# natir/yacrd

Hardware: AMD Instinct MI355X
Metric: reads_per_sec_classified (higher is better)
Workload: dtype u32

## Files before the change

include/yacrd_engine_debug.h:

```cpp
#ifndef YACRD_ENGINE_DEBUG_H
#define YACRD_ENGINE_DEBUG_H

#include "yacrd_engine.h"

#define YACRD_F_FORCE_GENERAL 1u
#define YACRD_F_FORCE_LDS_SORT 2u
#define YACRD_F_WAVE_ONLY 8u
#define YACRD_F_NO_HALVES 16u
#define YACRD_F_NO_PREDICTION 64u
#define YACRD_F_NO_PREFILTER 256u
#define YACRD_F_COUNT_PREFILTERED 512u
#define YACRD_F_NO_DEFER 4096u
#define YACRD_F_ALWAYS_DEFER 8192u
#define YACRD_F_SCREEN_ITEMS_1 262144u
#define YACRD_F_SCREEN_ITEMS_2 524288u
#define YACRD_F_NO_FUSED_SCREEN 1048576u
#define YACRD_F_STREAM_SCREEN 65536u
#define YACRD_F_SCREEN_WIDE 2097152u
#define YACRD_F_SCREEN_DIRECT 8388608u
#define YACRD_F_NO_SCREEN_DIRECT 16777216u

#ifdef __cplusplus
extern "C" {
#endif
int yacrd_debug_sort_pairs(yacrd_engine *e, uint64_t *keys, uint32_t *vals, uint64_t n, uint64_t key_bound);
uint64_t yacrd_debug_last_counters(const yacrd_engine *e, void *dst, uint64_t bytes);
int yacrd_debug_last_input_csr(yacrd_engine *e, uint64_t *n_reads, uint64_t *n_intervals, uint64_t *offsets, uint32_t *intervals,
                               uint32_t *lengths);
void yacrd_debug_peer_copy_counts(uint64_t out[3]);
void yacrd_debug_live_bytes(uint64_t out[2]);
uint64_t yacrd_debug_direct_runs(const yacrd_engine *e);
void yacrd_debug_big_routes(const yacrd_engine *e, uint64_t out[4]);
#ifdef __cplusplus
}
#endif

#endif
```

yacrd_amd/__init__.py:

```python
from .engine import (
    Engine, EngineError, NeedsHostParser, Result, lib_path, load_library, build, partition_reads, run_partitioned, ingest_overlaps,
    NOT_BAD, CHIMERIC, NOT_COVERED, TYPE_NAMES, F_FORCE_GENERAL, F_FORCE_LDS_SORT, F_WAVE_ONLY, F_NO_HALVES, F_TIMING_FULL, F_NO_PREDICTION, F_NO_PREFILTER, F_COUNT_PREFILTERED, F_NO_TIMING, F_BLOCKING_WAIT, F_NO_DEFER, F_ALWAYS_DEFER, F_TIMING_SAMPLED, F_STREAM_SCREEN, F_SCREEN_ITEMS_1, F_SCREEN_ITEMS_2, F_NO_FUSED_SCREEN, F_SCREEN_WIDE, F_ONE_LAUNCH, F_SCREEN_DIRECT, F_NO_SCREEN_DIRECT, DEBUG_SYMBOLS, run_device_batches, DeviceBatch,
    EXPORTED_SYMBOLS, CLASS_NAMES, CLASS_KERNELS, PinnedArray, Stream, StreamGroup, stream_device_of, HANDLE_ELSEWHERE, RecSink, OvlRec, OVL_REC_DTYPE, GzipWriter, ByteSink,
)
```

yacrd_amd/csrc/engine.hip:

```cpp
#include "engine_internal.h"

#include <time.h>

#include <algorithm>
#include <cstdio>
#include <cstdlib>
#include <cstring>
#include <string>
#include <thread>
#include <vector>

#include "device_common.h"
#include "plan_compact.h"
#include "sweep_big.h"
#include "sweep_wave.h"
#include "sweep_big_trim.h"
#include "sweep_general.h"
#include "sweep_lds.h"
#include "finish_compact.h"
#include "screen_wg.h"
#include "screen_stream.h"
#include "screen_big.h"
#include "one_batch.h"

using namespace yke;

static uint64_t env_u64(const char *name, uint64_t dflt)
{
    const char *v = std::getenv(name);
    return v ? std::strtoull(v, nullptr, 10) : dflt;
}

static uint64_t defer_min_intervals()
{
    static const uint64_t v = env_u64("YACRD_DEFER_MIN_IV", 4000000ull);
    return v;
}
static constexpr uint32_t kProbeEvery = 16;

static uint64_t split_min_reads()
{
    static const uint64_t v = env_u64("YACRD_SPLIT_MIN_READS", (uint64_t)yk::kPlanSmallReads);
    return v;
}

static uint64_t fused_share_override()
{
    static const uint64_t v = std::min<uint64_t>(env_u64("YACRD_FUSED_SHARE", 0), 4096);
    return v;
}
static uint64_t fused_grid_mult()
{
    static const uint64_t v = std::max<uint64_t>(1, env_u64("YACRD_TEST_FUSED_GRID_MULT", 1));
    return v;
}

namespace yke {
std::string &err_slot()
{
    thread_local std::string s;
    return s;
}
}

namespace {

yk::SweepArgs base_sweep_args(const yacrd_engine *e, const Run &R)
{
    yk::SweepArgs sa;
    sa.off = R.d_off, sa.iv = R.d_iv, sa.len = R.d_len, sa.cov = R.cov, sa.prefilter = R.prefilter;
    sa.list = nullptr, sa.list_n = nullptr, sa.rec = nullptr, sa.first = 0;
    sa.stage = e->stage.as<uint2>(), sa.counts = e->counts.as<u32>(), sa.closed = e->closed.as<uint2>(), sa.ctr = R.ctr;
    sa.rej_list = R.rej_small, sa.rej_count = &R.ctr->rej_small;
    sa.over_list = R.over_med, sa.over_count = &R.ctr->over_med;
    return sa;
}
yk::SweepArgs list_sweep_args(const Run &R, const u32 *list, const u32 *list_n)
{
    yk::SweepArgs sa = R.base;
    sa.list = list;
    sa.list_n = list_n;
    return sa;
}

yk::CompactArgs2 compact_args(const yacrd_engine *e, const Run &R)
{
    yk::CompactArgs2 ca;
    ca.sweep = R.base;
    ca.sweep.over_list = nullptr;
    ca.sweep.over_count = nullptr;
    ca.scan_state = reinterpret_cast<u64 *>(R.ctr + 1);
    ca.n_reads = R.n_reads;
    ca.not_cov = R.not_cov;
    ca.bad_offsets = e->bad_offsets.as<u64>();
    ca.bad_regions = e->bad_regions.as<uint2>();
    ca.region_cap = (u64)(e->bad_regions.cap / sizeof(uint2));
    ca.read_type = e->read_type.as<uint8_t>();
    ca.host_ctr = e->h_ctr();
    return ca;
}

int launch_compact(yacrd_engine *e, const Run &R)
{
    const u32 n_reads = R.n_reads;
    const yk::CompactArgs2 ca = compact_args(e, R);
    if (R.n_reads64 >= split_min_reads()) {
        if (R.screened) {
            const u32 slabs = (n_reads + yk::kMarkReads - 1) / yk::kMarkReads;
            yk::DeferList dl;
            dl.shard_cap = (slabs / yk::kDeferShards + 1u) * (u32)yk::kMarkReads;
            HIP_TRY(e->dlist.reserve((size_t)yk::kDeferShards * dl.shard_cap * sizeof(u32)));
            dl.list = e->dlist.as<u32>();
            dl.count = reinterpret_cast<u32 *>(ca.scan_state + R.nb);
            if (e->compact_calls++)
                HIP_TRY(hipMemsetAsync(dl.count, 0, (size_t)yk::kDeferShards * yk::kDeferShardStride * sizeof(u32), e->stream));
            hipLaunchKernelGGL(yk::mark_list_kernel, dim3(slabs), dim3(yk::kMarkThreads), 0, e->stream, ca.sweep.counts, n_reads, dl);
            hipLaunchKernelGGL(yk::deferred_list_kernel, dim3((u32)e->num_cu * (u32)(YK_LIST_OCC * 256 / yk::kListThreads)), dim3(yk::kListThreads), 0,
                               e->stream, ca.sweep, dl);
        }
        hipLaunchKernelGGL(yk::scan_compact_kernel<4>, dim3((n_reads + 4 * yk::kScanThreads - 1) / (4 * yk::kScanThreads)), dim3(yk::kScanThreads), 0, e->stream, ca);
        return YACRD_OK;
    }
    hipLaunchKernelGGL(yk::finish_compact_kernel, dim3((n_reads + yk::kScanBlock - 1) / yk::kScanBlock), dim3(yk::kScanBlock), 0, e->stream, ca);
    return YACRD_OK;
}

int gather_reads(yacrd_engine *e, const u64 *d_off, const u32 *d_len, const u32 *d_list, u32 count,
                 hipStream_t stream, std::vector<yk::GatherOut> &out)
{
    HIP_TRY(e->gen_sizes.reserve((size_t)count * sizeof(yk::GatherOut)));
    hipLaunchKernelGGL(yk::gather_general_sizes_kernel, dim3((count + 255) / 256), dim3(256), 0,
                       stream, d_off, d_len, d_list, count, e->gen_sizes.as<yk::GatherOut>());
    out.resize(count);
    HIP_TRY(hipMemcpyAsync(out.data(), e->gen_sizes.p, (size_t)count * sizeof(yk::GatherOut),
                           hipMemcpyDeviceToHost, stream));
    HIP_TRY(hipStreamSynchronize(stream));
    for (const auto &g : out)
        if (g.n >= 0x7FFFFFFFull) return fail(YACRD_EINVAL, "a read has >= 2^31 - 1 intervals");
    return YACRD_OK;
}

int run_general_global(yacrd_engine *e, const u64 *d_off, const uint2 *d_iv, const u32 *d_len,
                       const u32 *d_list, u32 count, u32 cov, hipStream_t stream)
{
    std::vector<yk::GatherOut> info;
    int rc = gather_reads(e, d_off, d_len, d_list, count, stream, info);
    if (rc) return rc;
    for (const auto &g : info)
        if (2 * g.n > (u64)yk::kMedium2Events) e->big_routes[3]++;
    HIP_TRY(e->gen_scratch_off.reserve((size_t)count * sizeof(u64)));
    std::vector<u64> offs(count);
    u64 tot = 0;
    for (u32 i = 0; i < count; i++) {
        offs[i] = tot;
        tot += 3 * info[i].n + 2;
    }
    HIP_TRY(e->gen_scratch.reserve((size_t)tot * sizeof(u64)));
    HIP_TRY(hipMemcpyAsync(e->gen_scratch_off.p, offs.data(), (size_t)count * sizeof(u64),
                           hipMemcpyHostToDevice, stream));
    HIP_TRY(hipStreamSynchronize(stream));
    yk::GeneralArgs ga;
    ga.off = d_off;
    ga.iv = d_iv;
    ga.len = d_len;
    ga.list = d_list;
    ga.scratch_off = e->gen_scratch_off.as<u64>();
    ga.scratch = e->gen_scratch.as<u64>();
    ga.cov = cov;
    ga.stage = e->stage.as<uint2>();
    ga.counts = e->counts.as<u32>();
    hipLaunchKernelGGL(yk::sweep_general_kernel, dim3(count), dim3(yk::kGenThreads), 0, stream, ga);
    return YACRD_OK;
}
// ... 129 lines not shown
        std::vector<yk::GatherOut> rest;
        for (u32 i = 0; i < count; i++) {
            if (bs[i].flags & yk::BT_TRIMMED) {
                e->big_routes[1]++;
                continue;
            }
            if (bs[i].flags & yk::BT_BAD) redo.push_back(info[i].read);
            else rest.push_back(info[i]);
        }
        info.swap(rest);
        count = (u32)info.size();
    }
    if (count) {
        rc = run_big_sort(e, d_iv, info, cov, stream, redo);
        if (rc) return rc;
    }
    if (!redo.empty()) {
        HIP_TRY(e->big_redo.reserve(redo.size() * sizeof(u32)));
        HIP_TRY(hipMemcpyAsync(e->big_redo.p, redo.data(), redo.size() * sizeof(u32),
                               hipMemcpyHostToDevice, stream));
        HIP_TRY(hipStreamSynchronize(stream));
        rc = run_general_global(e, d_off, d_iv, d_len, e->big_redo.as<u32>(), (u32)redo.size(), cov, stream);
        if (rc) return rc;
    }
    return YACRD_OK;
}

int wait_for_stream(yacrd_engine *e)
{
    if (e->flags & YACRD_F_BLOCKING_WAIT) {
        HIP_TRY(hipEventRecord(e->ev_sync[EVS_DONE], e->stream));
        for (;;) {
            const hipError_t q = hipEventQuery(e->ev_sync[EVS_DONE]);
            if (q == hipSuccess) break;
            if (q != hipErrorNotReady) HIP_TRY(q);
            struct timespec ts = {0, 20000};
            nanosleep(&ts, nullptr);
        }
    } else {
        HIP_TRY(hipStreamSynchronize(e->stream));
    }
    HIP_TRY(hipGetLastError());
    return YACRD_OK;
}

int conclude_run(yacrd_engine *e, const Run &R, float extra_ms);
int finish_pending(yacrd_engine *e);


int reserve_buffers(yacrd_engine *e, Run &R)
{
    const u32 n_reads = R.n_reads;
    const uint64_t n_reads64 = R.n_reads64;
    R.ob_slabs = (n_reads + yk::kObSlab - 1) / yk::kObSlab;
    R.nb = R.one_launch ? 2 * R.ob_slabs : (n_reads + yk::kScanBlock - 1) / yk::kScanBlock;
    constexpr int kLists = yk::CLS_COUNT + 9;
    HIP_TRY(e->lists.reserve((size_t)kLists * n_reads * sizeof(u32)));
    const size_t shard_ctr_bytes = (!R.one_launch && n_reads64 >= split_min_reads()) ? (size_t)yk::kDeferShards * yk::kDeferShardStride * sizeof(u32) : 0;
    R.ctrl_bytes = (sizeof(yk::Counters) + (size_t)R.nb * sizeof(u64) + shard_ctr_bytes + 255) & ~(size_t)255;
    e->compact_calls = 0;
    e->ctrl_cur ^= 1;
    const int cur = e->ctrl_cur, other = cur ^ 1;
    for (int i = 0; i < 2; i++) {
        const void *before = e->ctrl2[i].p;
        HIP_TRY(e->ctrl2[i].reserve(R.ctrl_bytes));
        if (e->ctrl2[i].p != before) e->ctrl_clean[i] = 0;
    }
    HIP_TRY(e->stage.reserve((size_t)(R.n_iv + 2 * n_reads64) * sizeof(uint2)));
    HIP_TRY(e->counts.reserve((size_t)n_reads * sizeof(u32)));
    HIP_TRY(e->closed.reserve((size_t)n_reads * sizeof(uint2)));
    HIP_TRY(e->read_type.reserve((size_t)n_reads));
    if (e->bad_regions.cap < (size_t)(4 * n_reads64 + 1024) * sizeof(uint2))
        HIP_TRY(e->bad_regions.reserve((size_t)(4 * n_reads64 + 1024) * sizeof(uint2)));

    R.mrec_cap1 = (u32)std::min<u64>(n_reads64, R.n_iv / 513 + 1), R.mrec_cap2 = (u32)std::min<u64>(n_reads64, R.n_iv / 4097 + 1);
    HIP_TRY(e->mrec.reserve(((size_t)R.mrec_cap1 + R.mrec_cap2) * sizeof(uint4)));
    R.lists = e->lists.as<u32>();
    e->last_list_stride = n_reads;
    R.rej_small = R.list_of(yk::CLS_COUNT), R.rej_med = R.list_of(yk::CLS_COUNT + 1);
    R.rej_big = R.list_of(yk::CLS_COUNT + 2), R.over_med = R.list_of(yk::CLS_COUNT + 3);
    R.fb_med[0] = R.list_of(yk::CLS_COUNT + 4), R.fb_med[1] = R.list_of(yk::CLS_COUNT + 5);
    R.fb_big = R.list_of(yk::CLS_COUNT + 6);
    R.fb_stream[0] = R.list_of(yk::CLS_COUNT + 7), R.fb_stream[1] = R.list_of(yk::CLS_COUNT + 8);
    R.ctr = e->ctrl2[cur].as<yk::Counters>();
    R.base = base_sweep_args(e, R);

    if (e->ctrl_clean[cur] < R.ctrl_bytes) HIP_TRY(hipMemsetAsync(R.ctr, 0, R.ctrl_bytes, e->stream));
    e->ctrl_clean[cur] = 0;
    R.other_bytes = std::min<size_t>(e->ctrl2[other].cap, (size_t)1 << 30) & ~(size_t)3;
    return YACRD_OK;
}

int launch_one_batch(yacrd_engine *e, Run &R)
{
    const int other = e->ctrl_cur ^ 1;
    yk::OneBatchArgs oa;
    oa.c = compact_args(e, R);
    oa.slab_ctr = oa.c.scan_state + R.ob_slabs;
    oa.n_slabs = R.ob_slabs;
    oa.zero = e->ctrl2[other].as<u32>();
    oa.zero_words = (u32)(R.other_bytes / 4);
    e->h_ctr()->ob_unsupported = 0;
    e->h_ctr()->scan_ticket = 0;
    hipLaunchKernelGGL(yk::one_batch_kernel, dim3(((R.ob_slabs + 7) / 8) * 8 * (u32)(yk::kObSlab / yk::kObReads)), dim3(64), 0, e->stream, oa);
    e->ctrl_clean[other] = R.other_bytes;
    if (R.full) HIP_TRY(hipEventRecord(e->ev[EV_COMPACT], e->stream));
    return YACRD_OK;
}

int launch_plan(yacrd_engine *e, Run &R)
{
// ... 467 lines not shown
    if (e->h_ctr()->rej_small > rej_small_done) return fail(YACRD_EINTERNAL, "rejected reads persisted");
    return YACRD_OK;
}

}

namespace yke {
static int rerun_without_fused(yacrd_engine *e, const Run R)
{
    e->fused_off = true;
    e->pred_valid = false;
    const int rc = run_on_device(e, R.d_off, R.d_iv, R.d_len, R.n_reads64, R.n_iv, R.cov, R.not_cov, false);
    e->fused_off = false;
    return rc;
}

static int hand_over(yacrd_engine *e, const Run &R, bool defer)
{
    e->pending = Pending{true, R.one_launch, R};
    return defer ? YACRD_OK : finish_pending(e);
}

int run_on_device(yacrd_engine *e, const u64 *d_off, const uint2 *d_iv, const u32 *d_len,
                  uint64_t n_reads64, uint64_t n_iv, uint32_t cov, double not_cov, bool defer)
{
    if (n_reads64 >= 0xFFFFFFFFull) return fail(YACRD_EINVAL, "n_reads must be < 2^32 - 1");
    if (e->pending.active) return fail(YACRD_EINVAL, "a submitted batch is pending: yacrd_engine_wait first");
    e->has_result = false;
    e->resident.valid = e->input.valid = false;
    e->timing = yacrd_timing{};
    for (uint64_t &r : e->big_routes) r = 0;

    HIP_TRY(e->bad_offsets.reserve((n_reads64 + 1) * sizeof(u64)));
    if (n_reads64 == 0) {
        HIP_TRY(hipMemsetAsync(e->bad_offsets.p, 0, sizeof(u64), e->stream));
        HIP_TRY(hipStreamSynchronize(e->stream));
        e->last_reads = 0;
        e->last_regions = 0;
        e->has_result = true;
        return YACRD_OK;
    }

    Run R;
    R.d_off = d_off, R.d_iv = d_iv, R.d_len = d_len;
    R.n_reads64 = n_reads64, R.n_reads = (u32)n_reads64, R.n_iv = n_iv, R.cov = cov, R.not_cov = not_cov;
    R.full = (e->flags & YACRD_F_TIMING_FULL) != 0;
    R.tight_grids = !(e->flags & YACRD_F_FORCE_LDS_SORT);
    R.prefilter = (e->flags & YACRD_F_NO_PREFILTER) ? 0u : (e->flags & YACRD_F_COUNT_PREFILTERED) ? 2u : 1u;
    for (int i = 0; i < 12; i++) R.cls_b[i] = R.cls_e[i] = -1;
    const uint64_t ob_waiters = (n_reads64 + yk::kObSlab - 1) / yk::kObSlab * 7 / 8;
    R.one_launch = (e->flags & YACRD_F_ONE_LAUNCH) && !e->one_launch_off && n_reads64 < (uint64_t)yk::kObMaxReads &&
                   e->num_xcc == 8 && 2 * ob_waiters <= (uint64_t)e->num_cu * 4 * YK_OB_OCC &&
                   !(e->flags & (YACRD_F_FORCE_GENERAL | YACRD_F_WAVE_ONLY | YACRD_F_FORCE_LDS_SORT | YACRD_F_NO_HALVES |
                                 YACRD_F_NO_PREFILTER | YACRD_F_NO_DEFER));

    int rc = reserve_buffers(e, R);
    if (rc) return rc;
    if (R.full) HIP_TRY(hipEventRecord(e->ev[EV_START], e->stream));
    if (R.one_launch) {
        rc = launch_one_batch(e, R);
        return rc ? rc : hand_over(e, R, defer);
    }
    R.timing_on = !(e->flags & YACRD_F_NO_TIMING);
    if ((e->flags & YACRD_F_TIMING_SAMPLED) && !R.full && (e->run_seq++ % 8u) != 0) R.timing_on = false;
    R.predicted = prediction_holds(e, R);
    R.direct = choose_direct(e, R);
    struct MissGuard {
        yacrd_engine *e;
        bool before;
        ~MissGuard() { e->miss_pending = before; }
    } miss_guard{e, e->miss_pending};
    struct SideGuard {
        yacrd_engine *e;
        const Run &R;
        bool joined = false;
        ~SideGuard()
        {
            if ((R.big_beside || R.direct) && !joined) (void)hipStreamSynchronize(e->side);
        }
    } side_guard{e, R};
    e->prev_build = e->last_build;
    e->last_build = -1;
    if (R.direct) {
        HIP_TRY(hipEventRecord(e->ev_sync[EVS_FORK], e->stream));
        if (R.full) HIP_TRY(hipEventRecord(e->ev[EV_S0], e->stream));
        launch_direct_screen(e, R);
        HIP_TRY(hipStreamWaitEvent(e->side, e->ev_sync[EVS_FORK], 0));
        rc = launch_plan(e, R);
        if (!rc) rc = size_launches(e, R);
        if (!rc) rc = launch_register_classes(e, R, R.ls, false);
        if (rc) return rc;
        HIP_TRY(hipEventRecord(e->ev_sync[EVS_JOIN], e->side));
        HIP_TRY(hipStreamWaitEvent(e->stream, e->ev_sync[EVS_JOIN], 0));
        side_guard.joined = true;
        if (R.full && R.timing_on) HIP_TRY(hipEventRecord(e->ev[EV_SMALL], e->stream));
        rc = launch_workgroup_classes(e, R, R.ls, false);
        if (!rc) launch_rejected_medium(e, R, R.ls);
        if (!rc) rc = join_device_wide_screen(e, R);
        if (rc) return rc;
    } else {
        rc = launch_plan(e, R);
        if (!rc) rc = size_launches(e, R);
        if (rc) return rc;
        if (R.full) HIP_TRY(hipEventRecord(e->ev[EV_S0], e->stream));
        rc = launch_device_wide_screen(e, R);
        if (!rc) rc = launch_sweeps(e, R, R.ls);
        if (!rc) rc = join_device_wide_screen(e, R);
// ... 770 lines not shown
```

yacrd_amd/csrc/finish_compact.h:

```cpp
#pragma once
#include "plan_compact.h"
#include "screen_reg.h"
#include "sweep_filtered.h"
#include "sweep_lds.h"
#include "sweep_wave.h"
#include "wave_ops.h"

namespace yk {

struct CompactArgs2 {
    SweepArgs sweep;
    u64 *scan_state;
    u32 n_reads;
    double not_cov;
    u64 *bad_offsets;
    uint2 *bad_regions;
    u64 region_cap;
    uint8_t *read_type;
    Counters *host_ctr;
};

constexpr int kFinishWaves = kScanBlock / 64;
#ifndef YK_FINISH_OCC
#define YK_FINISH_OCC 8
// ... 162 lines not shown
        }
        if (!fits) atomicOr(&ctr->region_overflow, 1u);
        c.read_type[r] = (uint8_t)classify(bad, middle, L, c.not_cov);
    }
}


#ifndef YK_DEFER_SWEEP_OCC
#define YK_DEFER_SWEEP_OCC 6
#endif

template <int LANES, int WPB, int TABW = kScreenTabWords>
__device__ __forceinline__ bool filtered_turn(const SweepArgs &a, bool active, u32 r, u64 o, u32 n, u32 len, const LaneConst &lc)
{
    constexpr int K = 16;
    const u32 lane = lane_id(), lig = lane & (u32)(LANES - 1);
    const i32 c = (i32)min(a.cov, 0x3FFFFFFFu);
    const bool two = active && n >= 2u;
    const uint2 *src = two ? a.iv + o : reinterpret_cast<const uint2 *>(a.off);
    const u32 last2 = two ? n - 2u : 0u;
    uint4 v[K / 4];
#pragma unroll
    for (int j = 0; j < K / 4; j++) v[j] = load_pair(src + min(2u * (lig + (u32)LANES * j), last2));
    u32 smin = v[0].x, emax = v[0].y, smax = v[0].x;
    i32 tmin = 0x7FFFFFFF;
#pragma unroll
    for (int j = 0; j < K / 4; j++) {
        smin = min(smin, min(v[j].x, v[j].z));
        smax = max(smax, max(v[j].x, v[j].z));
        emax = max(emax, max(v[j].y, v[j].w));
        tmin = min(tmin, min((i32)(v[j].y - v[j].x), (i32)(v[j].w - v[j].z)));
    }
    const int last_addr = (int)((lane | (u32)(LANES - 1)) << 2);
    const u32 pmin = (u32)__builtin_amdgcn_ds_bpermute(last_addr, (int)gscan_min<LANES>(smin));
    const u32 pmax = (u32)__builtin_amdgcn_ds_bpermute(last_addr, (int)gscan_max<LANES>(emax));
    const bool irregular = !two || pmax > min(len, kMaxKeyPos) || smax > kMaxKeyPos || tmin < (i32)kScreenWindow;
    const bool girr = group_any<LANES>(__builtin_amdgcn_ballot_w64(irregular));
    const u32 n_eff = girr ? 0u : n;
    bool real0[K / 4], real1[K / 4];
#pragma unroll
    for (int j = 0; j < K / 4; j++) {
        const u32 i0 = 2u * (lig + (u32)LANES * j);
        real0[j] = i0 + 1u < n_eff;
        real1[j] = i0 < n_eff;
    }
    return filtered_group_sweep<LANES, WPB, TABW>(a, v, real0, real1, r, o, n, len, c, pmin, pmax, !girr, lc);
}
constexpr u32 kDeferShards = 256, kDeferShardStride = 16;
struct DeferList {
    u32 *list;
    u32 *count;
    u32 shard_cap;
};
constexpr int kMarkThreads = 1024, kMarkReads = 4 * kMarkThreads;
__global__ __launch_bounds__(kMarkThreads) void mark_list_kernel(const u32 *__restrict__ counts, u32 n_reads, DeferList dl)
{
    __shared__ u32 s_ids[kMarkReads];
    __shared__ u32 s_n, s_base;
    if (threadIdx.x == 0) s_n = 0;
    __syncthreads();
    const u64 r0 = (u64)blockIdx.x * kMarkReads + threadIdx.x * 4u;
    u32 g[4] = {0, 0, 0, 0};
    if (r0 + 4 <= n_reads) {
        const uint4 g4 = *reinterpret_cast<const uint4 *>(counts + r0);
        g[0] = g4.x, g[1] = g4.y, g[2] = g4.z, g[3] = g4.w;
    } else {
#pragma unroll
        for (int k = 0; k < 4; k++) g[k] = r0 + k < n_reads ? counts[r0 + k] : 0u;
    }
    u32 mine = 0;
#pragma unroll
    for (int k = 0; k < 4; k++) mine += g[k] == kDeferredMark ? 1u : 0u;
    if (__builtin_amdgcn_ballot_w64(mine != 0) != 0) {
        u32 incl = mine;
#pragma unroll
        for (int d = 1; d < 64; d <<= 1) {
            const u32 t = (u32)__shfl_up((int)incl, d, 64);
            if ((int)lane_id() >= d) incl += t;
        }
        u32 base = 0;
        if (lane_id() == 63u) base = atomicAdd(&s_n, incl);
        base = (u32)__shfl((int)base, 63, 64);
        u32 at = base + incl - mine;
#pragma unroll
        for (int k = 0; k < 4; k++)
            if (g[k] == kDeferredMark) s_ids[at++] = (u32)(r0 + k);
    }
    __syncthreads();
    const u32 n = s_n;
    if (n == 0) return;
    const u32 shard = blockIdx.x & (kDeferShards - 1u);
    if (threadIdx.x == 0) s_base = atomicAdd(dl.count + shard * kDeferShardStride, n);
    __syncthreads();
    const u32 b0 = s_base;
    for (u32 i = threadIdx.x; i < n; i += kMarkThreads)
        if (b0 + i < dl.shard_cap) dl.list[(size_t)shard * dl.shard_cap + b0 + i] = s_ids[i];
}

#ifndef YK_LIST_THREADS
#define YK_LIST_THREADS 512
#endif
#ifndef YK_LIST_OCC
#define YK_LIST_OCC YK_DEFER_SWEEP_OCC
#endif
constexpr int kListThreads = YK_LIST_THREADS;
__global__ __launch_bounds__(kListThreads, YK_LIST_OCC) void deferred_list_kernel(SweepArgs a, DeferList dl)
{
    constexpr u32 kWaves = kListThreads / 64;
    constexpr int kTabWords = 2 * (2 * kScreenWindow + 32) * 4;
    static_assert(kDeferShards <= (u32)kListThreads, "one thread per shard counter");
    __shared__ u32 s_pre[kDeferShards + 1];
    __shared__ u32 sc[kWaves + 1];
    __shared__ uint4 s_list[kListThreads];
    __shared__ unsigned short s_fb[kListThreads];
    __shared__ u32 s_nfb;
    __shared__ unsigned long long s_iv;
    const u32 tid = threadIdx.x, lane = lane_id(), wv = tid >> 6;
    u32 total;
    {
        const u32 cnt = tid < kDeferShards ? min(dl.count[tid * kDeferShardStride], dl.shard_cap) : 0u;
        const u32 ex = block_excl_add<kListThreads>(cnt, sc, total);
        if (tid < kDeferShards) s_pre[tid] = ex;
        if (tid == 0) s_pre[kDeferShards] = total;
    }
    const u32 per = (total + gridDim.x - 1u) / gridDim.x;
    const u32 lo = (u32)min((u64)total, (u64)blockIdx.x * per), hi = (u32)min((u64)total, (u64)lo + per);
    if (lo >= hi) return;
    const LaneConst lcf = make_lane_const(lane);
    if (tid == 0) s_iv = 0;
    for (u32 c0 = lo; c0 < hi; c0 += (u32)kListThreads) {
        __syncthreads();
        if (tid == 0) s_nfb = 0;
        const u32 e = c0 + tid, n_here = min((u32)kListThreads, hi - c0);
        if (e < hi) {
            u32 s = 0;
#pragma unroll
            for (u32 step = kDeferShards / 2; step > 0; step >>= 1)
                if (s_pre[s + step] <= e) s += step;
            const u32 r = dl.list[(size_t)s * dl.shard_cap + (e - s_pre[s])];
            const u64 o = a.off[r];
            const u32 n = (u32)(a.off[r + 1] - o);
            s_list[tid] = make_uint4(r, n, a.len[r], 0u);
            atomicAdd(&s_iv, (unsigned long long)n);
        }
        __syncthreads();
        for (u32 p0 = wv * 2u; p0 < n_here; p0 += kWaves * 2u) {
            const u32 p = p0 + (lane >> 5);
            const bool have = p < n_here;
            const uint4 q = s_list[have ? p : p0];
            const u64 o = a.off[q.x];
            const bool done = filtered_turn<32, (int)kWaves, kTabWords>(a, have, q.x, o, q.y, q.z, lcf);
            if (have && !done && (lane & 31u) == 31u) s_fb[atomicAdd(&s_nfb, 1u)] = (unsigned short)p;
        }
        __syncthreads();
        const u32 nfb = s_nfb;
        for (u32 i = wv; i < nfb; i += kWaves) {
            const uint4 q = s_list[s_fb[i]];
            const u64 o = a.off[q.x];
            if (q.y > 128u) finish_item<8>(a.off, a.iv, a.len, a.stage, a.counts, a.rej_list, a.rej_count, a.ctr, a.cov, q.x, o, q.y, q.z);
            else finish_item<4>(a.off, a.iv, a.len, a.stage, a.counts, a.rej_list, a.rej_count, a.ctr, a.cov, q.x, o, q.y, q.z);
        }
    }
    __syncthreads();
    if (tid == 0) {
        atomicAdd((unsigned long long *)&a.ctr->deferred_iv, s_iv);
        atomicAdd(&a.ctr->deferred, hi - lo);
    }
}

constexpr int kScanThreads = 1024;
template <int PER>
__global__ __launch_bounds__(kScanThreads) void scan_compact_kernel(CompactArgs2 c)
{
    constexpr int kScanPer = PER, kScanReads = kScanThreads * PER;
    static_assert(PER % 4 == 0 && kScanReads % kScanBlock == 0, "16-byte loads; the control block holds one scan word per 1024 reads: more than this kernel's workgroups use");
    __shared__ u32 sc[kScanThreads / 64];
    __shared__ u32 s_bid;
    __shared__ u64 s_base;
    const SweepArgs &a = c.sweep;
    Counters *ctr = a.ctr;
    if (threadIdx.x == 0) s_bid = atomicAdd(&ctr->scan_ticket, 1u);
    __syncthreads();
    const u32 bid = s_bid, lane = lane_id();
    const u64 r0 = (u64)bid * kScanReads + threadIdx.x * (u32)kScanPer;
    u32 g[kScanPer], L[kScanPer];
    uint2 ab[kScanPer];
    bool closed[kScanPer];
    const bool vec = r0 + kScanPer <= c.n_reads && (reinterpret_cast<uintptr_t>(a.len) & 15u) == 0;
    if (vec) {
#pragma unroll
        for (int q = 0; q < kScanPer / 4; q++) {
            const uint4 g4 = *reinterpret_cast<const uint4 *>(a.counts + r0 + 4 * q);
            const uint4 l4 = *reinterpret_cast<const uint4 *>(a.len + r0 + 4 * q);
            g[4 * q] = g4.x, g[4 * q + 1] = g4.y, g[4 * q + 2] = g4.z, g[4 * q + 3] = g4.w;
            L[4 * q] = l4.x, L[4 * q + 1] = l4.y, L[4 * q + 2] = l4.z, L[4 * q + 3] = l4.w;
        }
    } else {
#pragma unroll
        for (int k = 0; k < kScanPer; k++) {
            const bool in = r0 + k < c.n_reads;
            g[k] = in ? a.counts[r0 + k] : 0u;
            L[k] = in ? a.len[r0 + k] : 0u;
        }
    }
    bool any_closed = false;
#pragma unroll
    for (int k = 0; k < kScanPer; k++) {
        if (g[k] == kDeferredMark) g[k] = 0u;
        closed[k] = g[k] == kClosedForm;
        any_closed |= closed[k];
        ab[k] = make_uint2(0u, L[k]);
    }
    if (any_closed) {
        if (vec) {
#pragma unroll
            for (int q = 0; q < kScanPer / 2; q++) {
                const uint4 c0 = *reinterpret_cast<const uint4 *>(a.closed + r0 + 2 * q);
                if (closed[2 * q]) ab[2 * q] = make_uint2(c0.x, c0.y);
                if (closed[2 * q + 1]) ab[2 * q + 1] = make_uint2(c0.z, c0.w);
            }
        } else {
#pragma unroll
            for (int k = 0; k < kScanPer; k++)
                if (closed[k]) ab[k] = a.closed[r0 + k];
        }
    }
    u32 mine = 0;
#pragma unroll
    for (int k = 0; k < kScanPer; k++) {
        if (closed[k]) g[k] = (ab[k].x != 0u ? 1u : 0u) + (ab[k].y != L[k] ? 1u : 0u);
        mine += g[k];
    }
    u32 tot;
    u32 local = block_excl_add<kScanThreads>(mine, sc, tot);
    if (threadIdx.x < 64) {
        constexpr u64 kAgg = 1ull << 62, kPre = 2ull << 62, kVal = (1ull << 62) - 1;
        u64 base = 0;
        if (bid > 0) {
            if (lane == 0) __hip_atomic_store(&c.scan_state[bid], kAgg | tot, __ATOMIC_RELAXED, __HIP_MEMORY_SCOPE_AGENT);
            for (i32 hi = (i32)bid - 1;; hi -= 64) {
                const i32 idx = hi - (i32)lane;
                u64 v, pre;
                for (;;) {
                    v = idx >= 0 ? __hip_atomic_load(&c.scan_state[idx], __ATOMIC_RELAXED, __HIP_MEMORY_SCOPE_AGENT) : kPre;
                    pre = __builtin_amdgcn_ballot_w64((v >> 62) == 2);
                    const u64 before = pre ? ((pre & (0 - pre)) - 1ull) : ~0ull;
                    if ((__builtin_amdgcn_ballot_w64((v >> 62) == 0) & before) == 0) break;
                    __builtin_amdgcn_s_sleep(1);
                }
                const u32 first_pre = pre ? (u32)__builtin_ctzll(pre) : 64u;
                u64 part = lane <= first_pre ? (v & kVal) : 0;
#pragma unroll
                for (int d = 32; d > 0; d >>= 1) part += __shfl_xor(part, d, 64);
                base += part;
                if (pre) break;
            }
        }
        if (lane == 0) {
            __hip_atomic_store(&c.scan_state[bid], kPre | (base + tot), __ATOMIC_RELAXED, __HIP_MEMORY_SCOPE_AGENT);
            s_base = base;
            if ((u64)(bid + 1) * kScanReads >= c.n_reads) ctr->total_regions = base + tot;
        }
        if (c.host_ctr && (u64)(bid + 1) * kScanReads >= c.n_reads) {
            const u64 total = (u64)__shfl((long long)(base + tot), 0, 64);
            const u32 *src = reinterpret_cast<const u32 *>(ctr);
            u32 *dst = reinterpret_cast<u32 *>(c.host_ctr);
            constexpr u32 kWords = (u32)(sizeof(Counters) / 4);
            for (u32 i = lane; i < kWords; i += 64u) {
                u32 w = __hip_atomic_load(&src[i], __ATOMIC_RELAXED, __HIP_MEMORY_SCOPE_AGENT);
                if (i == (u32)(offsetof(Counters, total_regions) / 4)) w = (u32)total;
                if (i == (u32)(offsetof(Counters, total_regions) / 4) + 1u) w = (u32)(total >> 32);
                if (i == (u32)(offsetof(Counters, region_overflow) / 4)) w = total > c.region_cap ? 1u : 0u;
                dst[i] = w;
            }
        }
    }
    __syncthreads();
    if (r0 >= c.n_reads) return;
    u64 dst = s_base + local;
    u64 offs[kScanPer];
    u64 types = 0;
    bool overflow = false;
#pragma unroll
    for (int k = 0; k < kScanPer; k++) {
        offs[k] = dst;
        const u64 r = r0 + k;
        if (r < c.n_reads) {
            u32 bad = 0;
            bool middle = false;
            const bool fits = dst + g[k] <= c.region_cap;
            if (closed[k]) {
                u32 j = 0;
                if (ab[k].x != 0u && fits) c.bad_regions[dst + j++] = make_uint2(0u, ab[k].x);
                if (ab[k].y != L[k] && fits) c.bad_regions[dst + j] = make_uint2(ab[k].y, L[k]);
                bad = ab[k].x + (L[k] - ab[k].y);
            } else if (g[k]) {
                const uint2 *slot = a.stage + (a.off[r] + 2 * r);
                for (u32 j = 0; j < g[k]; j++) {
                    const uint2 v = slot[j];
                    if (fits) c.bad_regions[dst + j] = v;
                    bad += v.y - v.x;
                    middle |= (v.x != 0u) & (v.y != L[k]);
                }
            }
            overflow |= !fits;
            types |= (u64)classify(bad, middle, L[k], c.not_cov) << (8 * k);
            if (r == c.n_reads - 1) c.bad_offsets[c.n_reads] = dst + g[k];
        }
        dst += g[k];
    }
    if (overflow) atomicOr(&ctr->region_overflow, 1u);
    if (r0 + kScanPer <= c.n_reads) {
        ulonglong2 *bo = reinterpret_cast<ulonglong2 *>(c.bad_offsets + r0);
#pragma unroll
        for (int q = 0; q < kScanPer / 2; q++) bo[q] = make_ulonglong2(offs[2 * q], offs[2 * q + 1]);
        if constexpr (kScanPer == 4) *reinterpret_cast<u32 *>(c.read_type + r0) = (u32)types;
        else *reinterpret_cast<u64 *>(c.read_type + r0) = types;
    } else {
#pragma unroll
        for (int k = 0; k < kScanPer; k++)
            if (r0 + k < c.n_reads) {
                c.bad_offsets[r0 + k] = offs[k];
                c.read_type[r0 + k] = (uint8_t)(types >> (8 * k));
            }
    }
}
// ... 3 lines not shown
```

yacrd_amd/engine.py:

```python
import ctypes
import os
import subprocess
from collections import namedtuple

import numpy as np

_HERE = os.path.dirname(os.path.abspath(__file__))
_LIB = os.path.join(_HERE, "lib", "libyacrd_hip.so")

NOT_BAD, CHIMERIC, NOT_COVERED = 0, 1, 2
TYPE_NAMES = {NOT_BAD: "NotBad", CHIMERIC: "Chimeric", NOT_COVERED: "NotCovered"}
F_FORCE_GENERAL = 1
F_FORCE_LDS_SORT = 2
F_WAVE_ONLY = 8
F_NO_HALVES = 16
F_TIMING_FULL = 32
F_NO_PREDICTION = 64
F_NO_PREFILTER = 256
F_COUNT_PREFILTERED = 512
F_NO_TIMING = 1024
F_BLOCKING_WAIT = 2048
F_NO_DEFER = 4096
F_ALWAYS_DEFER = 8192
F_TIMING_SAMPLED = 32768
F_STREAM_SCREEN = 65536
F_SCREEN_ITEMS_1 = 262144
F_SCREEN_ITEMS_2 = 524288
F_NO_FUSED_SCREEN = 1048576
F_SCREEN_WIDE = 2097152
F_SCREEN_DIRECT = 8388608
F_NO_SCREEN_DIRECT = 16777216
DEBUG_SYMBOLS = [
    "yacrd_debug_sort_pairs", "yacrd_debug_last_counters", "yacrd_debug_last_input_csr", "yacrd_debug_peer_copy_counts",
    "yacrd_debug_live_bytes", "yacrd_debug_direct_runs", "yacrd_debug_big_routes",
]
F_ONE_LAUNCH = 4194304

EXPORTED_SYMBOLS = [
    "yacrd_abi_version", "yacrd_last_error", "yacrd_engine_create", "yacrd_engine_destroy",
    "yacrd_engine_run", "yacrd_result_free", "yacrd_engine_run_device", "yacrd_engine_fetch",
    "yacrd_engine_last_timing", "yacrd_partition_reads", "yacrd_engine_classify",
    "yacrd_engines_run_partitioned", "yacrd_engine_timing_total", "yacrd_engine_event_overhead", "yacrd_engine_submit_device", "yacrd_engine_wait", "yacrd_engines_run_device_batches",
    "yacrd_engine_submit", "yacrd_engine_collect", "yacrd_pinned_alloc", "yacrd_pinned_free",
    "yacrd_stream_open", "yacrd_stream_sink", "yacrd_stream_acquire", "yacrd_stream_commit",
    "yacrd_stream_finish", "yacrd_stream_last_stats", "yacrd_stream_reset", "yacrd_stream_close",
    "yacrd_engine_ingest_paf", "yacrd_engine_ingest_overlaps", "yacrd_engine_ingest_overlaps_mem", "yacrd_engines_ingest_overlaps",
    "yacrd_engines_ingest_overlaps_mem", "yacrd_reads_free", "yacrd_engine_trim",
    "yacrd_engine_ingest_report", "yacrd_engine_ingest_report_mem", "yacrd_engine_write_report", "yacrd_engine_write_report_mem",
    "yacrd_engine_edit_overlaps", "yacrd_engine_edit_overlaps_mem", "yacrd_edit_text_free",
    "yacrd_engine_edit_overlaps_gzip_mem", "yacrd_engine_edit_overlaps_gzip_file",
    "yacrd_engine_edit_fastq", "yacrd_engine_edit_fastq_mem", "yacrd_engine_edit_fastq_gzip_mem", "yacrd_engine_edit_fastq_gzip_file",
    "yacrd_engine_edit_fasta", "yacrd_engine_edit_fasta_mem", "yacrd_engine_edit_fasta_gzip_mem", "yacrd_engine_edit_fasta_gzip_file",
    "yacrd_engine_gunzip_mem", "yacrd_engine_edit_fastq_bgzf_mem", "yacrd_engine_edit_fastq_bgzf_file",
    "yacrd_engine_edit_fasta_bgzf_mem", "yacrd_engine_edit_fasta_bgzf_file",
    "yacrd_engine_gzip_mem", "yacrd_gzip_writer_open", "yacrd_gzip_writer_write", "yacrd_gzip_writer_sink", "yacrd_gzip_writer_close",
    "yacrd_gzip_writer_abort",
    "yacrd_stream_device_of", "yacrd_stream_group_open", "yacrd_stream_group_sink", "yacrd_stream_group_finish",
    "yacrd_stream_group_last_stats", "yacrd_stream_group_reset", "yacrd_stream_group_close",
]


class EngineError(RuntimeError):
    pass


class NeedsHostParser(EngineError):
    """yacrd_engine_ingest_paf returned YACRD_EFALLBACK: the input is for the host parser."""


E_FALLBACK = 5


class _Reads(ctypes.Structure):
    _fields_ = [("n_reads", ctypes.c_uint64), ("n_records", ctypes.c_uint64),
                ("lengths", ctypes.POINTER(ctypes.c_uint32)), ("name_off", ctypes.POINTER(ctypes.c_uint64)),
                ("names", ctypes.POINTER(ctypes.c_char))]


class _ReportTable(ctypes.Structure):
    _fields_ = [("n_reads", ctypes.c_uint64)] + \
               [(n, ctypes.c_void_p) for n in ("name_off", "names", "lengths", "bad_offsets", "bad_regions", "read_type")]


class _ReportWriteStats(ctypes.Structure):
# ... 1086 lines not shown
```

Baseline: 3.449 billion.

## Replace decoupled look-back scan with precomputed slab/super-slab region sums

The mark_list_kernel now counts the regions in each 4096-read slab. The deferred_list kernel adds its finished reads' counts into per-slab and per-super-slab totals. scan_compact_kernel then computes each workgroup's base by summing these precomputed prefixes, instead of using an atomic ticket and a serial decoupled look-back chain. This removes the inter-workgroup spin-waiting. The cost is that mark_list_kernel always runs on the split path, reads the closed/len arrays, and uses extra atomics. A new flag forces the split path, and the scan kernel gets an occupancy hint in its launch bounds.

```diff
diff --git a/include/yacrd_engine_debug.h b/include/yacrd_engine_debug.h
--- a/include/yacrd_engine_debug.h
+++ b/include/yacrd_engine_debug.h
@@ -19,6 +19,7 @@
 #define YACRD_F_SCREEN_WIDE 2097152u
 #define YACRD_F_SCREEN_DIRECT 8388608u
 #define YACRD_F_NO_SCREEN_DIRECT 16777216u
+#define YACRD_F_SPLIT_FOLLOW_ON 33554432u
 
 #ifdef __cplusplus
 extern "C" {
diff --git a/yacrd_amd/__init__.py b/yacrd_amd/__init__.py
--- a/yacrd_amd/__init__.py
+++ b/yacrd_amd/__init__.py
@@ -1,5 +1,5 @@
 from .engine import (
     Engine, EngineError, NeedsHostParser, Result, lib_path, load_library, build, partition_reads, run_partitioned, ingest_overlaps,
-    NOT_BAD, CHIMERIC, NOT_COVERED, TYPE_NAMES, F_FORCE_GENERAL, F_FORCE_LDS_SORT, F_WAVE_ONLY, F_NO_HALVES, F_TIMING_FULL, F_NO_PREDICTION, F_NO_PREFILTER, F_COUNT_PREFILTERED, F_NO_TIMING, F_BLOCKING_WAIT, F_NO_DEFER, F_ALWAYS_DEFER, F_TIMING_SAMPLED, F_STREAM_SCREEN, F_SCREEN_ITEMS_1, F_SCREEN_ITEMS_2, F_NO_FUSED_SCREEN, F_SCREEN_WIDE, F_ONE_LAUNCH, F_SCREEN_DIRECT, F_NO_SCREEN_DIRECT, DEBUG_SYMBOLS, run_device_batches, DeviceBatch,
+    NOT_BAD, CHIMERIC, NOT_COVERED, TYPE_NAMES, F_FORCE_GENERAL, F_FORCE_LDS_SORT, F_WAVE_ONLY, F_NO_HALVES, F_TIMING_FULL, F_NO_PREDICTION, F_NO_PREFILTER, F_COUNT_PREFILTERED, F_NO_TIMING, F_BLOCKING_WAIT, F_NO_DEFER, F_ALWAYS_DEFER, F_TIMING_SAMPLED, F_STREAM_SCREEN, F_SCREEN_ITEMS_1, F_SCREEN_ITEMS_2, F_NO_FUSED_SCREEN, F_SCREEN_WIDE, F_ONE_LAUNCH, F_SCREEN_DIRECT, F_NO_SCREEN_DIRECT, F_SPLIT_FOLLOW_ON, DEBUG_SYMBOLS, run_device_batches, DeviceBatch,
     EXPORTED_SYMBOLS, CLASS_NAMES, CLASS_KERNELS, PinnedArray, Stream, StreamGroup, stream_device_of, HANDLE_ELSEWHERE, RecSink, OvlRec, OVL_REC_DTYPE, GzipWriter, ByteSink,
 )
diff --git a/yacrd_amd/csrc/engine.hip b/yacrd_amd/csrc/engine.hip
--- a/yacrd_amd/csrc/engine.hip
+++ b/yacrd_amd/csrc/engine.hip
@@ -43,6 +43,11 @@
     static const uint64_t v = env_u64("YACRD_SPLIT_MIN_READS", (uint64_t)yk::kPlanSmallReads);
     return v;
 }
+static bool split_follow_on(const yacrd_engine *e, uint64_t n_reads)
+{
+    return (e->flags & YACRD_F_SPLIT_FOLLOW_ON) || n_reads >= split_min_reads();
+}
+static uint32_t split_slabs(uint32_t n_reads) { return (n_reads + (uint32_t)yk::kMarkReads - 1) / (uint32_t)yk::kMarkReads; }
 
 static uint64_t fused_share_override()
 {
@@ -104,21 +109,24 @@
 {
     const u32 n_reads = R.n_reads;
     const yk::CompactArgs2 ca = compact_args(e, R);
-    if (R.n_reads64 >= split_min_reads()) {
+    if (split_follow_on(e, R.n_reads64)) {
+        const u32 slabs = split_slabs(n_reads);
+        const yk::SlabSums ss = yk::slab_sums(R.ctr);
+        yk::DeferList dl{};
         if (R.screened) {
-            const u32 slabs = (n_reads + yk::kMarkReads - 1) / yk::kMarkReads;
-            yk::DeferList dl;
             dl.shard_cap = (slabs / yk::kDeferShards + 1u) * (u32)yk::kMarkReads;
             HIP_TRY(e->dlist.reserve((size_t)yk::kDeferShards * dl.shard_cap * sizeof(u32)));
             dl.list = e->dlist.as<u32>();
             dl.count = reinterpret_cast<u32 *>(ca.scan_state + R.nb);
             if (e->compact_calls++)
                 HIP_TRY(hipMemsetAsync(dl.count, 0, (size_t)yk::kDeferShards * yk::kDeferShardStride * sizeof(u32), e->stream));
-            hipLaunchKernelGGL(yk::mark_list_kernel, dim3(slabs), dim3(yk::kMarkThreads), 0, e->stream, ca.sweep.counts, n_reads, dl);
+        }
+        hipLaunchKernelGGL(yk::mark_list_kernel, dim3(slabs), dim3(yk::kMarkThreads), 0, e->stream, ca.sweep.counts, ca.sweep.closed, ca.sweep.len,
+                           n_reads, dl, ss, R.screened ? 1u : 0u);
+        if (R.screened)
             hipLaunchKernelGGL(yk::deferred_list_kernel, dim3((u32)e->num_cu * (u32)(YK_LIST_OCC * 256 / yk::kListThreads)), dim3(yk::kListThreads), 0,
                                e->stream, ca.sweep, dl);
-        }
-        hipLaunchKernelGGL(yk::scan_compact_kernel<4>, dim3((n_reads + 4 * yk::kScanThreads - 1) / (4 * yk::kScanThreads)), dim3(yk::kScanThreads), 0, e->stream, ca);
+        hipLaunchKernelGGL(yk::scan_compact_kernel<4>, dim3(slabs), dim3(yk::kScanThreads), 0, e->stream, ca);
         return YACRD_OK;
     }
     hipLaunchKernelGGL(yk::finish_compact_kernel, dim3((n_reads + yk::kScanBlock - 1) / yk::kScanBlock), dim3(yk::kScanBlock), 0, e->stream, ca);
@@ -354,11 +362,12 @@
 {
     const u32 n_reads = R.n_reads;
     const uint64_t n_reads64 = R.n_reads64;
+    const bool split = !R.one_launch && split_follow_on(e, n_reads64);
     R.ob_slabs = (n_reads + yk::kObSlab - 1) / yk::kObSlab;
-    R.nb = R.one_launch ? 2 * R.ob_slabs : (n_reads + yk::kScanBlock - 1) / yk::kScanBlock;
+    R.nb = R.one_launch ? 2 * R.ob_slabs : split ? yk::kMaxSupers + split_slabs(n_reads) : (n_reads + yk::kScanBlock - 1) / yk::kScanBlock;
     constexpr int kLists = yk::CLS_COUNT + 9;
     HIP_TRY(e->lists.reserve((size_t)kLists * n_reads * sizeof(u32)));
-    const size_t shard_ctr_bytes = (!R.one_launch && n_reads64 >= split_min_reads()) ? (size_t)yk::kDeferShards * yk::kDeferShardStride * sizeof(u32) : 0;
+    const size_t shard_ctr_bytes = split ? (size_t)yk::kDeferShards * yk::kDeferShardStride * sizeof(u32) : 0;
     R.ctrl_bytes = (sizeof(yk::Counters) + (size_t)R.nb * sizeof(u64) + shard_ctr_bytes + 255) & ~(size_t)255;
     e->compact_calls = 0;
     e->ctrl_cur ^= 1;
@@ -932,7 +941,7 @@
     R.one_launch = (e->flags & YACRD_F_ONE_LAUNCH) && !e->one_launch_off && n_reads64 < (uint64_t)yk::kObMaxReads &&
                    e->num_xcc == 8 && 2 * ob_waiters <= (uint64_t)e->num_cu * 4 * YK_OB_OCC &&
                    !(e->flags & (YACRD_F_FORCE_GENERAL | YACRD_F_WAVE_ONLY | YACRD_F_FORCE_LDS_SORT | YACRD_F_NO_HALVES |
-                                 YACRD_F_NO_PREFILTER | YACRD_F_NO_DEFER));
+                                 YACRD_F_NO_PREFILTER | YACRD_F_NO_DEFER | YACRD_F_SPLIT_FOLLOW_ON));
 
     int rc = reserve_buffers(e, R);
     if (rc) return rc;
diff --git a/yacrd_amd/csrc/finish_compact.h b/yacrd_amd/csrc/finish_compact.h
--- a/yacrd_amd/csrc/finish_compact.h
+++ b/yacrd_amd/csrc/finish_compact.h
@@ -238,25 +238,67 @@
     u32 *count;
     u32 shard_cap;
 };
+constexpr u32 kSuperShift = 10;
+constexpr u32 kMaxSupers = 1024;
+struct SlabSums {
+    u64 *super;
+    u64 *slab;
+};
+__host__ __device__ __forceinline__ SlabSums slab_sums(Counters *ctr)
+{
+    SlabSums ss;
+    ss.super = reinterpret_cast<u64 *>(ctr + 1), ss.slab = ss.super + kMaxSupers;
+    return ss;
+}
 constexpr int kMarkThreads = 1024, kMarkReads = 4 * kMarkThreads;
-__global__ __launch_bounds__(kMarkThreads) void mark_list_kernel(const u32 *__restrict__ counts, u32 n_reads, DeferList dl)
+__global__ __launch_bounds__(kMarkThreads) void mark_list_kernel(const u32 *__restrict__ counts, const uint2 *__restrict__ closed,
+                                                                 const u32 *__restrict__ len, u32 n_reads, DeferList dl, SlabSums ss, u32 list)
 {
     __shared__ u32 s_ids[kMarkReads];
     __shared__ u32 s_n, s_base;
+    __shared__ u64 s_sum[kMarkThreads / 64];
     if (threadIdx.x == 0) s_n = 0;
     __syncthreads();
     const u64 r0 = (u64)blockIdx.x * kMarkReads + threadIdx.x * 4u;
     u32 g[4] = {0, 0, 0, 0};
-    if (r0 + 4 <= n_reads) {
+    const bool whole = r0 + 4 <= n_reads;
+    if (whole) {
         const uint4 g4 = *reinterpret_cast<const uint4 *>(counts + r0);
         g[0] = g4.x, g[1] = g4.y, g[2] = g4.z, g[3] = g4.w;
     } else {
 #pragma unroll
         for (int k = 0; k < 4; k++) g[k] = r0 + k < n_reads ? counts[r0 + k] : 0u;
     }
+    u64 regions = 0;
+    bool any_closed = false;
+#pragma unroll
+    for (int k = 0; k < 4; k++) {
+        if (g[k] < kClosedForm) regions += g[k];
+        any_closed |= g[k] == kClosedForm;
+    }
+    if (any_closed) {
+        if (whole && (reinterpret_cast<uintptr_t>(len) & 15u) == 0) {
+            const uint4 l4 = *reinterpret_cast<const uint4 *>(len + r0);
+            const uint4 c0 = *reinterpret_cast<const uint4 *>(closed + r0), c1 = *reinterpret_cast<const uint4 *>(closed + r0 + 2);
+            if (g[0] == kClosedForm) regions += (c0.x != 0u ? 1u : 0u) + (c0.y != l4.x ? 1u : 0u);
+            if (g[1] == kClosedForm) regions += (c0.z != 0u ? 1u : 0u) + (c0.w != l4.y ? 1u : 0u);
+            if (g[2] == kClosedForm) regions += (c1.x != 0u ? 1u : 0u) + (c1.y != l4.z ? 1u : 0u);
+            if (g[3] == kClosedForm) regions += (c1.z != 0u ? 1u : 0u) + (c1.w != l4.w ? 1u : 0u);
+        } else {
+#pragma unroll
+            for (int k = 0; k < 4; k++)
+                if (g[k] == kClosedForm) {
+                    const uint2 ab = closed[r0 + k];
+                    regions += (ab.x != 0u ? 1u : 0u) + (ab.y != len[r0 + k] ? 1u : 0u);
+                }
+        }
+    }
+#pragma unroll
+    for (int d = 32; d > 0; d >>= 1) regions += __shfl_xor(regions, d, 64);
+    if (lane_id() == 0) s_sum[threadIdx.x >> 6] = regions;
     u32 mine = 0;
 #pragma unroll
-    for (int k = 0; k < 4; k++) mine += g[k] == kDeferredMark ? 1u : 0u;
+    for (int k = 0; k < 4; k++) mine += (list && g[k] == kDeferredMark) ? 1u : 0u;
     if (__builtin_amdgcn_ballot_w64(mine != 0) != 0) {
         u32 incl = mine;
 #pragma unroll
@@ -273,6 +315,13 @@
             if (g[k] == kDeferredMark) s_ids[at++] = (u32)(r0 + k);
     }
     __syncthreads();
+    if (threadIdx.x == 0) {
+        u64 t = 0;
+#pragma unroll
+        for (int w = 0; w < kMarkThreads / 64; w++) t += s_sum[w];
+        ss.slab[blockIdx.x] = t;
+        if (t) atomicAdd((unsigned long long *)&ss.super[blockIdx.x >> kSuperShift], (unsigned long long)t);
+    }
     const u32 n = s_n;
     if (n == 0) return;
     const u32 shard = blockIdx.x & (kDeferShards - 1u);
@@ -301,6 +350,8 @@
     __shared__ unsigned short s_fb[kListThreads];
     __shared__ u32 s_nfb;
     __shared__ unsigned long long s_iv;
+    __shared__ unsigned long long s_sup;
+    __shared__ u32 s_sup_key;
     const u32 tid = threadIdx.x, lane = lane_id(), wv = tid >> 6;
     u32 total;
     {
@@ -327,6 +378,7 @@
             const u64 o = a.off[r];
             const u32 n = (u32)(a.off[r + 1] - o);
             s_list[tid] = make_uint4(r, n, a.len[r], 0u);
+            if (e == lo) s_sup = 0, s_sup_key = r / (u32)kMarkReads >> kSuperShift;
             atomicAdd(&s_iv, (unsigned long long)n);
         }
         __syncthreads();
@@ -346,29 +398,59 @@
             if (q.y > 128u) finish_item<8>(a.off, a.iv, a.len, a.stage, a.counts, a.rej_list, a.rej_count, a.ctr, a.cov, q.x, o, q.y, q.z);
             else finish_item<4>(a.off, a.iv, a.len, a.stage, a.counts, a.rej_list, a.rej_count, a.ctr, a.cov, q.x, o, q.y, q.z);
         }
+        __syncthreads();
+        if (c0 + (tid & ~63u) < hi) {
+            const bool have = c0 + tid < hi;
+            const u32 r = have ? s_list[tid].x : 0u;
+            u32 g = have ? __hip_atomic_load(&a.counts[r], __ATOMIC_RELAXED, __HIP_MEMORY_SCOPE_AGENT) : 0u;
+            if (g >= kClosedForm) g = 0u;
+            const u32 slab = have ? r / (u32)kMarkReads : ~0u;
+            const u32 prev = (u32)__shfl_up((int)slab, 1, 64);
+            const bool first = lane == 0u || prev != slab;
+            const u64 heads = __builtin_amdgcn_ballot_w64(first);
+            const u64 above = lane == 63u ? 0ull : heads & ~((2ull << lane) - 1ull);
+            const u32 last = above ? (u32)__builtin_ctzll(above) - 1u : 63u;
+            const u32 incl = wave_incl_add(g);
+            const u32 sum = (u32)__shfl((int)incl, (int)last, 64) - incl + g;
+            if (first && have && sum != 0u) {
+                const SlabSums ss = slab_sums(a.ctr);
+                atomicAdd((unsigned long long *)&ss.slab[slab], (unsigned long long)sum);
+                const u32 sup = slab >> kSuperShift;
+                if (sup == s_sup_key) atomicAdd(&s_sup, (unsigned long long)sum);
+                else atomicAdd((unsigned long long *)&ss.super[sup], (unsigned long long)sum);
+            }
+        }
     }
     __syncthreads();
     if (tid == 0) {
+        if (s_sup) atomicAdd((unsigned long long *)&slab_sums(a.ctr).super[s_sup_key], s_sup);
         atomicAdd((unsigned long long *)&a.ctr->deferred_iv, s_iv);
         atomicAdd(&a.ctr->deferred, hi - lo);
     }
 }
 
 constexpr int kScanThreads = 1024;
+#ifndef YK_SCAN_OCC
+#define YK_SCAN_OCC 8
+#endif
 template <int PER>
-__global__ __launch_bounds__(kScanThreads) void scan_compact_kernel(CompactArgs2 c)
+__global__ __launch_bounds__(kScanThreads, YK_SCAN_OCC) void scan_compact_kernel(CompactArgs2 c)
 {
     constexpr int kScanPer = PER, kScanReads = kScanThreads * PER;
-    static_assert(PER % 4 == 0 && kScanReads % kScanBlock == 0, "16-byte loads; the control block holds one scan word per 1024 reads: more than this kernel's workgroups use");
+    static_assert(PER % 4 == 0, "16-byte loads");
+    static_assert(kScanReads == kMarkReads, "a scan workgroup's reads are one slab of mark_list_kernel: its sum is this workgroup's");
+    static_assert((1u << kSuperShift) <= (u32)kScanThreads && kMaxSupers <= (u32)kScanThreads, "one thread per slab of the open super slab, one per super slab in front");
     __shared__ u32 sc[kScanThreads / 64];
-    __shared__ u32 s_bid;
+    __shared__ u64 s_pre[kScanThreads / 64];
     __shared__ u64 s_base;
     const SweepArgs &a = c.sweep;
     Counters *ctr = a.ctr;
-    if (threadIdx.x == 0) s_bid = atomicAdd(&ctr->scan_ticket, 1u);
-    __syncthreads();
-    const u32 bid = s_bid, lane = lane_id();
+    const SlabSums ss = slab_sums(ctr);
+    const u32 bid = blockIdx.x, lane = lane_id();
     const u64 r0 = (u64)bid * kScanReads + threadIdx.x * (u32)kScanPer;
+    const u32 n_sup = bid >> kSuperShift, n_open = bid & ((1u << kSuperShift) - 1u);
+    u64 pre = threadIdx.x < n_sup ? ss.super[threadIdx.x] : 0;
+    if (threadIdx.x < n_open) pre += ss.slab[(n_sup << kSuperShift) + threadIdx.x];
     u32 g[kScanPer], L[kScanPer];
     uint2 ab[kScanPer];
     bool closed[kScanPer];
@@ -417,47 +499,33 @@
         if (closed[k]) g[k] = (ab[k].x != 0u ? 1u : 0u) + (ab[k].y != L[k] ? 1u : 0u);
         mine += g[k];
     }
+    if ((threadIdx.x & ~63u) < max(n_sup, n_open)) {
+#pragma unroll
+        for (int d = 32; d > 0; d >>= 1) pre += __shfl_xor(pre, d, 64);
+    }
+    if (lane == 0) s_pre[threadIdx.x >> 6] = pre;
     u32 tot;
-    u32 local = block_excl_add<kScanThreads>(mine, sc, tot);
+    const u32 local = block_excl_add<kScanThreads>(mine, sc, tot);
+    static_assert(kScanThreads / 64 == 16, "one partial per lane of a group of sixteen");
     if (threadIdx.x < 64) {
-        constexpr u64 kAgg = 1ull << 62, kPre = 2ull << 62, kVal = (1ull << 62) - 1;
-        u64 base = 0;
-        if (bid > 0) {
-            if (lane == 0) __hip_atomic_store(&c.scan_state[bid], kAgg | tot, __ATOMIC_RELAXED, __HIP_MEMORY_SCOPE_AGENT);
-            for (i32 hi = (i32)bid - 1;; hi -= 64) {
-                const i32 idx = hi - (i32)lane;
-                u64 v, pre;
-                for (;;) {
-                    v = idx >= 0 ? __hip_atomic_load(&c.scan_state[idx], __ATOMIC_RELAXED, __HIP_MEMORY_SCOPE_AGENT) : kPre;
-                    pre = __builtin_amdgcn_ballot_w64((v >> 62) == 2);
-                    const u64 before = pre ? ((pre & (0 - pre)) - 1ull) : ~0ull;
-                    if ((__builtin_amdgcn_ballot_w64((v >> 62) == 0) & before) == 0) break;
-                    __builtin_amdgcn_s_sleep(1);
+        u64 base = s_pre[lane & 15u];
+#pragma unroll
+        for (int d = 8; d > 0; d >>= 1) base += __shfl_xor(base, d, 64);
+        if (lane == 0) s_base = base;
+        if ((u64)(bid + 1) * kScanReads >= c.n_reads) {
+            const u64 total = base + tot;
+            if (lane == 0) __hip_atomic_store(&ctr->total_regions, total, __ATOMIC_RELAXED, __HIP_MEMORY_SCOPE_AGENT);
+            if (c.host_ctr) {
+                const u32 *src = reinterpret_cast<const u32 *>(ctr);
+                u32 *dst = reinterpret_cast<u32 *>(c.host_ctr);
+                constexpr u32 kWords = (u32)(sizeof(Counters) / 4);
+                for (u32 i = lane; i < kWords; i += 64u) {
+                    u32 w = __hip_atomic_load(&src[i], __ATOMIC_RELAXED, __HIP_MEMORY_SCOPE_AGENT);
+                    if (i == (u32)(offsetof(Counters, total_regions) / 4)) w = (u32)total;
+                    if (i == (u32)(offsetof(Counters, total_regions) / 4) + 1u) w = (u32)(total >> 32);
+                    if (i == (u32)(offsetof(Counters, region_overflow) / 4)) w = total > c.region_cap ? 1u : 0u;
+                    __hip_atomic_store(&dst[i], w, __ATOMIC_RELAXED, __HIP_MEMORY_SCOPE_SYSTEM);
                 }
-                const u32 first_pre = pre ? (u32)__builtin_ctzll(pre) : 64u;
-                u64 part = lane <= first_pre ? (v & kVal) : 0;
-#pragma unroll
-                for (int d = 32; d > 0; d >>= 1) part += __shfl_xor(part, d, 64);
-                base += part;
-                if (pre) break;
-            }
-        }
-        if (lane == 0) {
-            __hip_atomic_store(&c.scan_state[bid], kPre | (base + tot), __ATOMIC_RELAXED, __HIP_MEMORY_SCOPE_AGENT);
-            s_base = base;
-            if ((u64)(bid + 1) * kScanReads >= c.n_reads) ctr->total_regions = base + tot;
-        }
-        if (c.host_ctr && (u64)(bid + 1) * kScanReads >= c.n_reads) {
-            const u64 total = (u64)__shfl((long long)(base + tot), 0, 64);
-            const u32 *src = reinterpret_cast<const u32 *>(ctr);
-            u32 *dst = reinterpret_cast<u32 *>(c.host_ctr);
-            constexpr u32 kWords = (u32)(sizeof(Counters) / 4);
-            for (u32 i = lane; i < kWords; i += 64u) {
-                u32 w = __hip_atomic_load(&src[i], __ATOMIC_RELAXED, __HIP_MEMORY_SCOPE_AGENT);
-                if (i == (u32)(offsetof(Counters, total_regions) / 4)) w = (u32)total;
-                if (i == (u32)(offsetof(Counters, total_regions) / 4) + 1u) w = (u32)(total >> 32);
-                if (i == (u32)(offsetof(Counters, region_overflow) / 4)) w = total > c.region_cap ? 1u : 0u;
-                dst[i] = w;
             }
         }
     }
diff --git a/yacrd_amd/engine.py b/yacrd_amd/engine.py
--- a/yacrd_amd/engine.py
+++ b/yacrd_amd/engine.py
@@ -30,6 +30,7 @@
 F_SCREEN_WIDE = 2097152
 F_SCREEN_DIRECT = 8388608
 F_NO_SCREEN_DIRECT = 16777216
+F_SPLIT_FOLLOW_ON = 33554432
 DEBUG_SYMBOLS = [
     "yacrd_debug_sort_pairs", "yacrd_debug_last_counters", "yacrd_debug_last_input_csr", "yacrd_debug_peer_copy_counts",
     "yacrd_debug_live_bytes", "yacrd_debug_direct_runs", "yacrd_debug_big_routes",
```

Result: slower. 3.315 billion (-3.9%).
